# smolGura/fish-tts

Hardware: AMD Instinct MI355X
Metric: semantic tokens/sec (higher is better)
Workload: dtype bf16; 1 GPU; openaudio-s1-mini shapes (BASELINE configs[1]): batch=1 per GPU, 48-token prompt, 215 frames (10 s), top-p sampling, hipGraph-captured frame step, + DAC codec decode; prompt_len=48, parallelism=replica x1, frame_engine=3

## Files before the change

### fish-tts_amd/_lib.py

```python
from __future__ import annotations

import ctypes as C
import os
import subprocess

_HERE = os.path.dirname(os.path.abspath(__file__))
CSRC = os.path.join(_HERE, "csrc")
LIB_PATH = os.path.join(CSRC, "libfishtts_hip.so")

FT_OK = 0
FT_ERR_ARG, FT_ERR_HIP, FT_ERR_STATE, FT_ERR_UNSUPPORTED, FT_ERR_NOMEM, FT_ERR_TOO_LONG, FT_ERR_MISSING_WEIGHT = range(1, 8)
FT_F32, FT_BF16, FT_F16 = 0, 1, 2


class ft_ar_config(C.Structure):
    _fields_ = [(n, C.c_int32) for n in ("dtype", "vocab_size", "n_layer", "n_head", "dim", "intermediate_size",
                                         "n_local_heads", "head_dim")] + \
               [("rope_base", C.c_float), ("norm_eps", C.c_float)] + \
               [(n, C.c_int32) for n in ("max_seq_len", "tie_word_embeddings", "attention_qkv_bias", "attention_o_bias",
                                         "attention_qk_norm", "codebook_size", "num_codebooks",
                                         "scale_codebook_embeddings", "n_fast_layer", "fast_dim", "fast_n_head",
                                         "fast_n_local_heads", "fast_head_dim", "fast_intermediate_size",
                                         "fast_attention_qkv_bias", "fast_attention_qk_norm", "fast_attention_o_bias",
                                         "semantic_begin_id", "semantic_end_id", "im_end_id", "max_batch",
# ... 32 lines not shown
    "ft_ar_prefill_slow_many": (C.c_int32, [_P, C.c_int32, _P, _P, _P, _P]),
    "ft_ar_prefill_at": (C.c_int32, [_P, C.c_int32, _P, C.c_int32, C.c_int32, C.POINTER(ft_sampling), _P]),
    "ft_ar_kv_save": (C.c_int32, [_P, C.c_int32, C.c_int32, C.POINTER(_P)]),
    "ft_ar_kv_restore": (C.c_int32, [_P, _P, C.c_int32]),
    "ft_ar_kv_positions": (C.c_int32, [_P]),
    "ft_ar_kv_free": (None, [_P, _P]),
    "ft_ar_decode": (C.c_int32, [_P, C.c_int32, C.c_int32, C.POINTER(ft_sampling), C.c_int32, _P, _P]),
    "ft_ar_set_noise": (C.c_int32, [_P, _P, C.c_int64, C.c_int64]),
    "ft_ar_get_debug": (C.c_int32, [_P, C.c_int32, _P, _P]),
    "ft_codec_decode": (C.c_int32, [_P, _P, C.c_int32, C.c_int32, _P, _P]),
    "ft_codec_frame_len": (C.c_int32, [_P]),
    "ft_codec_stream_begin": (C.c_int32, [_P, C.POINTER(_P)]),
    "ft_codec_stream_decode": (C.c_int32, [_P, _P, _P, C.c_int32, _P]),
    "ft_codec_stream_end": (None, [_P, _P]),
    "ft_codec_stream_decode_many": (C.c_int32, [_P, C.c_int32, _P, _P, _P, _P]),
    "ft_resample_filter": (C.c_int32, [C.c_int32, _P, _P, _P, _P]),
    "ft_resampled_len": (C.c_int64, [C.c_int32, C.c_int64]),
    "ft_codec_decode_at": (C.c_int32, [_P, _P, C.c_int32, C.c_int32, _P, C.c_int32, _P, _P]),
    "ft_codec_stream_begin_at": (C.c_int32, [_P, C.c_int32, C.POINTER(_P)]),
    "ft_codec_stream_decode_many_at": (C.c_int32, [_P, C.c_int32, _P, _P, _P, _P, _P, _P]),
    "ft_test_resample": (C.c_int32, [_P, _P, C.c_int64, C.c_int32, _P, _P]),
    "ft_codec_encode": (C.c_int32, [_P, _P, C.c_int64, _P, _P]),
    "ft_codec_enc_frame_len": (C.c_int32, [_P]),
    "ft_codec_rvq_encode": (C.c_int32, [_P, _P, C.c_int32, _P]),
    "ft_ar_profile_gemv": (C.c_int32, [_P, C.c_int32, C.POINTER(ft_sampling), C.POINTER(C.c_double),
                                       C.POINTER(C.c_int64), C.POINTER(C.c_int64)]),
    "ft_ar_profile_frame": (C.c_int32, [_P, C.c_int32, C.POINTER(ft_sampling), C.POINTER(C.c_double), C.POINTER(C.c_double),
                                        C.POINTER(C.c_int32)]),
    "ft_sync": (C.c_int32, [_P]),
    "ft_ar_engine_state": (C.c_int32, [_P, _P, _P, _P]),
    "ft_ar_frame_path": (C.c_char_p, [_P]),
    "ft_test_engine_fault": (C.c_int32, [_P, C.c_int32, C.c_int32, C.c_int32]),
    "ft_test_sample": (C.c_int32, [_P, _P, C.c_int32, C.POINTER(ft_sampling), _P, _P, _P]),
    "ft_test_codec_trace_arm": (C.c_int32, [_P, C.c_int32, C.c_int32]),
    "ft_test_codec_trace_count": (C.c_int32, [_P]),
    "ft_test_codec_trace_variants": (C.c_int32, []),
    "ft_test_codec_trace_variant": (C.c_char_p, [C.c_int32, C.POINTER(C.c_int32), C.POINTER(C.c_int32)]),
    "ft_test_codec_trace_launch": (C.c_int32, [_P, C.c_int32, C.c_char_p, C.c_int32, C.POINTER(C.c_int32)]),
    "ft_test_codec_trace_buffer": (C.c_int32, [_P, C.c_int32, C.c_int32, C.POINTER(C.c_int32), C.POINTER(C.c_int32),
                                               C.POINTER(C.c_int64), _P]),
}

HIPCC_FLAGS = ["-O3", "--offload-arch=gfx950", "-ffp-contract=off", "-fPIC", "-shared", "-std=c++17",
               "-Wno-unused-value"]
SOURCES = ["engine.hip", "codec.hip"]


def _deps(path: str, seen=None) -> set:
    seen = set() if seen is None else seen
    path = os.path.normpath(path)
    if path in seen or not os.path.exists(path):
        return seen
    seen.add(path)
    with open(path) as f:
        for line in f:
            if line.startswith("#include \""):
                _deps(os.path.join(os.path.dirname(path), line.split('"')[1]), seen)
    return seen


def build(force: bool = False) -> str:
    hipcc = os.environ.get("HIPCC", "/opt/rocm/bin/hipcc")
    flags = [f for f in HIPCC_FLAGS if f != "-shared"]
    jobs, objs = [], []
    for s in SOURCES:
        src, obj = os.path.join(CSRC, s), os.path.join(CSRC, s.replace(".hip", ".o"))
# ... 35 lines not shown
```

### fish-tts_amd/ar_engine.py

```python
from __future__ import annotations

import ctypes as C
import logging
from typing import Dict, Iterator, List, Optional, Sequence

import numpy as np
import torch

from . import _lib as L
from .config import DualARModelArgs


class HipError(RuntimeError):
    pass


logger = logging.getLogger(__name__)


def _rope_table(n_pos: int, n_elem: int, base: float) -> torch.Tensor:
    expo = torch.arange(0, n_elem, 2)[: n_elem // 2].float() / n_elem
    inv_freq = 1.0 / (base ** expo)
    ang = torch.outer(torch.arange(n_pos), inv_freq)
    z = torch.polar(torch.ones_like(ang), ang)
# ... 201 lines not shown
        arr = (L.ft_sampling * ns)(*samplings)
        frames = np.zeros((ns, max(n_frames, 1), self.R), dtype=np.int32)
        n = np.zeros(ns, dtype=np.int32)
        self._check(self.lib.ft_ar_decode(self._h, ns, n_frames, arr, poll, frames.ctypes.data_as(C.c_void_p),
                                          n.ctypes.data_as(C.c_void_p)), "ft_ar_decode")
        return frames, n

    def set_noise(self, q: Optional[np.ndarray]):
        if q is None:
            self._check(self.lib.ft_ar_set_noise(self._h, None, 0, 0), "ft_ar_set_noise")
            return
        q = np.ascontiguousarray(q, dtype=np.float32)
        self._check(self.lib.ft_ar_set_noise(self._h, q.ctypes.data_as(C.c_void_p), q.shape[0], q.shape[1]),
                    "ft_ar_set_noise")

    def debug_state(self, slot: int = 0):
        logits = np.zeros(self.args.vocab_size, dtype=np.float32)
        hidden = np.zeros(self.args.fast_dim, dtype=np.float32)
        self._check(self.lib.ft_ar_get_debug(self._h, slot, logits.ctypes.data_as(C.c_void_p),
                                             hidden.ctypes.data_as(C.c_void_p)), "ft_ar_get_debug")
        return logits, hidden

    def test_sample(self, logits: np.ndarray, cb: int, sampling: L.ft_sampling, window=None, q=None) -> int:
        logits = np.ascontiguousarray(logits, dtype=np.float32)
        w = None if window is None else np.ascontiguousarray(window, dtype=np.int32)
        qq = None if q is None else np.ascontiguousarray(q, dtype=np.float32)
        out = np.zeros(1, dtype=np.int32)
        self._check(self.lib.ft_test_sample(
            self._h, logits.ctypes.data_as(C.c_void_p), cb, C.byref(sampling),
            None if w is None else w.ctypes.data_as(C.c_void_p),
            None if qq is None else qq.ctypes.data_as(C.c_void_p), out.ctypes.data_as(C.c_void_p)), "ft_test_sample")
        return int(out[0])

    def engine_state(self):
        f, a, w = C.c_int32(0), C.c_int32(0), C.c_int32(0)
        self._check(self.lib.ft_ar_engine_state(self._h, C.byref(f), C.byref(a), C.byref(w)), "ft_ar_engine_state")
        return f.value, a.value, w.value

    def sync(self):
        self._check(self.lib.ft_sync(self._h), "ft_sync")

    def profile_gemv(self, frames: int, sampling: L.ft_sampling):
        ms, n, b = C.c_double(), C.c_int64(), C.c_int64()
        self._check(self.lib.ft_ar_profile_gemv(self._h, frames, C.byref(sampling), C.byref(ms), C.byref(n),
                                                C.byref(b)), "ft_ar_profile_gemv")
        return ms.value, n.value, b.value

    def profile_frame(self, frames: int, sampling: L.ft_sampling):
        ms, n = C.c_double(0), C.c_int32(0)
        seg = (C.c_double * 3)()
        self._check(self.lib.ft_ar_profile_frame(self._h, frames, C.byref(sampling), C.byref(ms), seg, C.byref(n)),
                    "ft_ar_profile_frame")
        return ms.value, [seg[0], seg[1], seg[2]], n.value

    def _clamp_new(self, T: int, max_new_tokens: int) -> int:
        m = self.args.max_seq_len
        if T >= m:
            raise ValueError(f"Input sequence length {T} exceeds max_seq_len {m}")
        if max_new_tokens:
            if T + max_new_tokens > m:
                max_new_tokens = m - T
        else:
            max_new_tokens = m - T
        return min(max_new_tokens, self.max_new_tokens)

    def generate(self, prompt: np.ndarray, max_new_tokens: int, temperature: float = 0.7, top_p: float = 0.7,
# ... 45 lines not shown
```

### fish-tts_amd/csrc/ar_kernels.h

```cpp
#pragma once
#include "common.h"

namespace ft {

enum { PRO_NONE = 0, PRO_RMSNORM = 1 };
enum { EPI_STORE = 0, EPI_RESID = 1, EPI_SWIGLU = 2 };

__device__ __host__ __forceinline__ size_t xo_index(int m, int k, int ldm) { return ((size_t)(k >> 3) * ldm + m) * 8 + (k & 7); }

struct GemvP {
    const void* W;
    const void* bias;
    const float* x;
    int ldx;
    const void* gain;
    float eps;
    float* out;
    int ldo;
    const float* resid;
    int ldr;
    int N, K;
    int pro, epi;
    int nt;
};
// ... 1416 lines not shown
        const float* qrow = nullptr;
        if (p.noise && nfv < p.noise_rows) qrow = p.noise + (size_t)nfv * p.noise_row_len + p.noise_off;
        float q4[4];
        draw_noise4(p, ctl, qrow, i0, nfv, m, V, q4);
        ArgMax best{-1.f, 0x7fffffff};
#pragma unroll
        for (int e = 0; e < 4; ++e) {
            if (i0 + e < V) {
                const float prob = keep[e] ? rb<ROUND>(et[e] / Z2) : 0.f;
                best = better(best, ArgMax{rb<ROUND>(prob / rb<ROUND>(q4[e])), i0 + e});
            }
        }
        winner = block_best(best).i;
    }
    __syncthreads();
    finish_draw<WT>(p, m, winner, nfv);
}

struct SampCut {
    unsigned kstar;
    int nk;
    int all_kept;
    int argmax;
    float Lmax, Mt, Z2, Tc;
};

struct SampBigP {
    SampP s;
    SampCut* cut;
    int* chunk_cnt;
    float* part_score;
    int* part_idx;
    int nchunk;
};

__device__ __forceinline__ float key16_value(unsigned k16) {
    const uint32_t k = k16 << 16;
    const uint32_t u = (k & 0x80000000u) ? (k & 0x7fffffffu) : ~(k | 0xffffu);
    return __uint_as_float(u);
}

constexpr int SAMP_TH_THREADS = 1024;
constexpr int SAMP_TH_ROW = 33;
constexpr int SAMP_TH_OVF = 8;
constexpr size_t SAMP_TH_LDS = (size_t)SAMP_TH_THREADS * SAMP_TH_ROW * 4;

struct SampThShared {
    float red[16];
    int redi[16];
    float wsum[16];
    int wact[16];
    int AL[1024];
    unsigned ovf_key[SAMP_TH_OVF];
    unsigned ovf_cnt[SAMP_TH_OVF];
    int ovf_n;
    SampCut cut_s;
};

__device__ __forceinline__ void samp_cut_from_image(const SampBigP& b, const int m, const uint32_t* cimg, SampThShared& sh,
                                                    const bool has, const int kmax_t) {
    const SampP& p = b.s;
    const int tid = threadIdx.x, lane = tid & 63, wave = tid >> 6;
    const RowCtl ctl = p.ctl[m];
    float* red = sh.red;
    int* redi = sh.redi;
    float* wsum = sh.wsum;
    int* wact = sh.wact;
    int* AL = sh.AL;
    unsigned* ovf_key = sh.ovf_key;
    unsigned* ovf_cnt = sh.ovf_cnt;
    int& ovf_n = sh.ovf_n;
    SampCut& cut_s = sh.cut_s;
    const unsigned long long hb = __ballot(has);
    if (lane == 0) wact[wave] = __popcll(hb);
    __syncthreads();
    int abase = 0, n_active = 0;
    for (int w = 0; w < 16; ++w) { if (w < wave) abase += wact[w]; n_active += wact[w]; }
    if (has) AL[abase + __popcll(hb & ((1ull << lane) - 1ull))] = tid;
    ArgMax km = block_argmax(ArgMax{(float)kmax_t, tid}, red, redi);
    const unsigned kmax = (unsigned)(int)km.v;
    const float Lmax = key16_value(kmax);
    const int n_items = n_active * 64;
    const int ipt = (n_items + 1023) / 1024;
    const int i0 = tid * ipt, i1 = min(i0 + ipt, n_items);
    auto item_count = [&](int i, unsigned& k) -> float {
        const int g = AL[i >> 6], j = i & 63;
        k = 64u * g + j;
        const uint32_t w = cimg[g * SAMP_TH_ROW + (j >> 1)];
        unsigned c = (j & 1) ? (w >> 16) : (w & 0xffffu);
        if (c == 65535u)
            for (int q = 0; q < ovf_n && q < SAMP_TH_OVF; ++q) if (ovf_key[q] == k) c = ovf_cnt[q];
        return (float)c;
    };
    float z = 0.f;
    for (int i = i0; i < i1; ++i) {
        unsigned k;
        const float c = item_count(i, k);
        if (c > 0.f) z = fmaf(c, expf(key16_value(k) - Lmax), z);
    }
    const float Z = block_sum(z, red);
    const float tp = round_bf16(ctl.top_p);
    auto removed = [&](float cum) { return round_bf16(cum) > tp; };
    auto prob = [&](unsigned k16) { return round_bf16(expf(key16_value(k16) - Lmax) / Z); };
    float mt = 0.f;
    for (int i = i0; i < i1; ++i) {
        unsigned k;
        const float c = item_count(i, k);
        if (c > 0.f) mt = fmaf(c, prob(k), mt);
    }
    float suf = mt;
#pragma unroll
    for (int o = 1; o < 64; o <<= 1) {
        const float t = __shfl_down(suf, o, 64);
        if (lane + o < 64) suf += t;
    }
    __syncthreads();
    if (lane == 0) wsum[wave] = suf;
    __syncthreads();
    float above = suf - mt;
    for (int w = wave + 1; w < 16; ++w) above += wsum[w];
    int found = -1;
    unsigned f_key = 0;
    float f_above = 0.f, f_cnt = 0.f;
    float run = above;
    for (int i = i1 - 1; i >= i0; --i) {
        unsigned k;
        const float c = item_count(i, k);
        if (c > 0.f) {
            const float nxt = fmaf(c, prob(k), run);
            if (found < 0 && removed(nxt)) { found = i; f_key = k; f_above = run; f_cnt = c; }
            run = nxt;
        }
    }
    ArgMax who = block_argmax(ArgMax{found >= 0 ? (float)tid : -1.f, tid}, red, redi);
    if (tid == 0) { cut_s.all_kept = who.v < 0.f ? 1 : 0; cut_s.kstar = 0; cut_s.nk = 0; }
    __syncthreads();
    if (who.v >= 0.f && tid == (int)who.v) {
        const float pk = prob(f_key);
        int lo_n = 0, hi_n = (int)f_cnt;
        while (lo_n < hi_n) {
            const int mid = (lo_n + hi_n + 1) >> 1;
            if (removed(fmaf((float)mid, pk, f_above))) hi_n = mid - 1; else lo_n = mid;
        }
        if (f_key == kmax && lo_n < 1) lo_n = 1;
        cut_s.kstar = f_key;
        cut_s.nk = lo_n;
    }
    __syncthreads();
    const unsigned kstar = cut_s.kstar;
    const int nk = cut_s.nk, all_kept = cut_s.all_kept;
    const float Tc = fmaxf(ctl.temperature, 1e-5f);
    const float Mt = round_bf16(Lmax / Tc);
    float z2 = 0.f;
    for (int i = i0; i < i1; ++i) {
        unsigned k;
        const float c = item_count(i, k);
        if (c > 0.f) {
            float n = 0.f;
            if (all_kept || k > kstar) n = c;
            else if (k == kstar) n = (float)nk;
            if (n > 0.f) z2 = fmaf(n, expf(round_bf16(key16_value(k) / Tc) - Mt), z2);
        }
    }
    const float Z2 = block_sum(z2, red);
    if (tid == 0) {
        SampCut o;
        o.kstar = kstar; o.nk = nk; o.all_kept = all_kept; o.argmax = 0;
        o.Lmax = Lmax; o.Mt = Mt; o.Z2 = Z2; o.Tc = Tc;
        b.cut[m] = o;
    }
}

static __global__ __launch_bounds__(1024) void samp_cut_kernel(SampBigP b) {
    extern __shared__ __attribute__((aligned(16))) uint32_t cimg[];
    __shared__ SampThShared sh;
    __shared__ int pen_id[32];
    __shared__ float pen_val[32];
    const SampP& p = b.s;
    const int m = blockIdx.x, tid = threadIdx.x;
    float* L = p.logits + (size_t)m * p.ldl;
    const int V = p.V;
    const RowCtl ctl = p.ctl[m];
    const int nfv = p.nf[m];
    const int R = p.ncb + 1;
    const int* seq = p.seq + (size_t)m * R * p.cap;
    for (int i = tid; i < SAMP_TH_THREADS * SAMP_TH_ROW; i += 1024) cimg[i] = 0u;
    if (tid == 0) sh.ovf_n = 0;
    const int npen = nfv > 0 ? (p.cb == 0 ? R : 16) : 0;
    auto count1 = [&](float v) {
        const unsigned k = order_key(v) >> 16;
        atomicAdd(&cimg[(k >> 6) * SAMP_TH_ROW + ((k & 63u) >> 1)], (k & 1u) ? 0x10000u : 1u);
    };
    {
        if (nfv > 0) {
            const int it = nfv - 1;
            const int ws = it < 16 ? 0 : it - 16;
            if (tid < npen) {
                const int id = p.cb == 0 ? seq[(size_t)tid * p.cap + ws + 1] : seq[(size_t)(p.cb + 1) * p.cap + ws + 1 + tid];
                pen_id[tid] = -1;
                if (id >= 0 && id < V) {
                    const float sv = L[id];
                    pen_id[tid] = id;
                    pen_val[tid] = sv < 0.f ? round_bf16(sv * ctl.rep) : round_bf16(sv / ctl.rep);
                }
            }
            __syncthreads();
            if (tid < npen && pen_id[tid] >= 0) L[pen_id[tid]] = pen_val[tid];
        }
        if (p.cb == 0 && ctl.ban_eos && tid == 0 && p.im_end < V) L[p.im_end] = -INFINITY;
        __syncthreads();
        const int V16 = ((reinterpret_cast<uintptr_t>(L) & 15) == 0) ? (V / 16384) * 16384 : 0;
        float4 fa[4], fb[4];
        auto ld16 = [&](float4 (&f)[4], int base) {
#pragma unroll
            for (int u = 0; u < 4; ++u) f[u] = *reinterpret_cast<const float4*>(L + base + u * 4096 + tid * 4);
        };
        auto cnt16 = [&](const float4 (&f)[4]) {
#pragma unroll
            for (int u = 0; u < 4; ++u) { count1(f[u].x); count1(f[u].y); count1(f[u].z); count1(f[u].w); }
        };
        if (V16 > 0) ld16(fa, 0);
        for (int base = 0; base < V16; base += 32768) {
            if (base + 16384 < V16) ld16(fb, base + 16384);
            cnt16(fa);
            if (base + 32768 < V16) ld16(fa, base + 32768);
            if (base + 16384 < V16) cnt16(fb);
        }
        for (int base = V16; base < V; base += 4096) {
            float f[4];
#pragma unroll
            for (int u = 0; u < 4; ++u) { const int i = base + u * 1024 + tid; f[u] = i < V ? L[i] : 0.f; }
#pragma unroll
            for (int u = 0; u < 4; ++u) if (base + u * 1024 + tid < V) count1(f[u]);
        }
    }
    __syncthreads();
    const uint32_t* row = cimg + tid * SAMP_TH_ROW;
    int kmax_t = -1;
    unsigned tot = 0;
#pragma unroll 8
    for (int j = 0; j < 32; ++j) {
        const uint32_t w = row[j];
        const unsigned c0 = w & 0xffffu, c1 = w >> 16;
        if (c0) kmax_t = 64 * tid + 2 * j;
        if (c1) kmax_t = 64 * tid + 2 * j + 1;
        tot += c0 + c1;
    }
    const int total = (int)block_sum((float)tot, sh.red);
    if (total != V) {
        __shared__ unsigned exc_key[SAMP_TH_OVF];
        __shared__ unsigned exc_cnt[SAMP_TH_OVF];
        for (int i = tid; i < SAMP_TH_THREADS * SAMP_TH_ROW; i += 1024) cimg[i] = 0u;
        if (tid < SAMP_TH_OVF) { exc_key[tid] = 0xffffffffu; exc_cnt[tid] = 0u; }
        __syncthreads();
        for (int i = tid; i < V; i += 1024) {
            const unsigned k = order_key(L[i]) >> 16;
            uint32_t* d = &cimg[(k >> 6) * SAMP_TH_ROW + ((k & 63u) >> 1)];
            const unsigned shft = (k & 1u) * 16u;
            for (;;) {
                const uint32_t old = *reinterpret_cast<volatile uint32_t*>(d);
                if (((old >> shft) & 0xffffu) == 65535u) {
                    for (int q = 0; q < SAMP_TH_OVF; ++q) {
                        const unsigned prev = atomicCAS(&exc_key[q], 0xffffffffu, k);
                        if (prev == 0xffffffffu || prev == k) { atomicAdd(&exc_cnt[q], 1u); break; }
                    }
                    break;
                }
                if (atomicCAS(d, old, old + (1u << shft)) == old) break;
            }
        }
        __syncthreads();
        if (tid == 0) {
            int n = 0;
            for (int q = 0; q < SAMP_TH_OVF; ++q)
                if (exc_key[q] != 0xffffffffu) { sh.ovf_key[n] = exc_key[q]; sh.ovf_cnt[n] = 65535u + exc_cnt[q]; ++n; }
            sh.ovf_n = n;
        }
        kmax_t = -1;
        tot = 0;
        for (int j = 0; j < 32; ++j) {
            const uint32_t w = row[j];
            if (w & 0xffffu) kmax_t = 64 * tid + 2 * j;
            if (w >> 16) kmax_t = 64 * tid + 2 * j + 1;
            tot += (w & 0xffffu) + (w >> 16);
        }
        __syncthreads();
    }
    samp_cut_from_image(b, m, cimg, sh, tot != 0u, kmax_t);
}

static __global__ __launch_bounds__(256) void samp_count_kernel(SampBigP b) {
    __shared__ float red[4];
    const SampP& p = b.s;
    const int m = blockIdx.y, tid = threadIdx.x;
    const int c0 = blockIdx.x * 1024;
    const float* L = p.logits + (size_t)m * p.ldl;
    const SampCut cut = b.cut[m];
    float c = 0.f;
#pragma unroll
    for (int e = 0; e < 4; ++e) {
        const int i = c0 + 4 * tid + e;
        if (i < p.V && (order_key(L[i]) >> 16) == cut.kstar) c += 1.f;
    }
    c = wave_sum(c);
    if ((tid & 63) == 0) red[tid >> 6] = c;
    __syncthreads();
    if (tid == 0) b.chunk_cnt[(size_t)m * b.nchunk + blockIdx.x] = (int)(red[0] + red[1] + red[2] + red[3]);
}

static __global__ __launch_bounds__(256) void samp_race_kernel(SampBigP b) {
    __shared__ float red[4];
    __shared__ int redi[4];
    __shared__ int wcnt[4];
    const SampP& p = b.s;
    const int m = blockIdx.y, tid = threadIdx.x, lane = tid & 63, wave = tid >> 6;
    const int c0 = blockIdx.x * 1024;
    const float* L = p.logits + (size_t)m * p.ldl;
    const int V = p.V;
    const RowCtl ctl = p.ctl[m];
    const int nfv = p.nf[m];
// ... 74 lines not shown
```

### fish-tts_amd/csrc/engine.h

```cpp
#pragma once
#include <hip/hip_runtime.h>

#include <map>
#include <string>
#include <vector>

#include "../../include/fishtts_hip.h"
#include "../../include/fishtts_hip_test.h"
#include "common.h"

namespace ft {
struct RowCtl;
struct SampCut;
struct EngLayer;
}

struct FtTensor {
    void* p = nullptr;
    std::vector<int64_t> shape;
    int dtype = FT_BF16;
    int64_t numel() const {
        int64_t n = 1;
        for (auto s : shape) n *= s;
        return n;
// ... 28 lines not shown
    std::vector<FtLayer> layers, flayers;

    float *x = nullptr, *qkv = nullptr, *y = nullptr, *g = nullptr, *logits = nullptr, *hid = nullptr,
          *femb = nullptr, *xf = nullptr, *qkvf = nullptr, *gf = nullptr, *flog = nullptr, *part_o = nullptr,
          *part_ml = nullptr;
    int n_slots = 0, nsplit = 1, cap = 0, fastV = 0, y_ld = 0;
    int nsplit_max = 1;
    bool nsplit_fixed = false;
    float *pf_x = nullptr, *pf_qkv = nullptr, *pf_y = nullptr;
    ft::bf16_t *pf_xn = nullptr, *pf_ybf = nullptr, *pf_g = nullptr, *pf_qbf = nullptr;
    int4* pf_seqs = nullptr;
    int2* pf_rows = nullptr;
    ft::bf16_t *xo_x = nullptr, *xo_xf = nullptr, *xo_femb = nullptr, *xo_y = nullptr, *xo_g = nullptr;
    ft::bf16_t* wide_qkv0_tab = nullptr;
    int xo_ldm = 0;
    int xo_pair = 0;
    bool no_attn_wide = false;
    bool no_head_stream = false;
    bool no_pair = false;
    int wide_min = 5;
    bool wide_ok = false;
    bool prefill_v0 = false;
    int prefill_gemm_mode = 2;
    size_t cache_m_stride = 0, fcache_m_stride = 0;

    int *d_pos = nullptr, *d_tok = nullptr, *d_tokn = nullptr, *d_seq = nullptr, *d_nf = nullptr,
        *d_done = nullptr, *d_prompt = nullptr;
    ft::RowCtl* d_ctl = nullptr;
    int *h_pin = nullptr;
    float* noise = nullptr;
    long noise_rows = 0, noise_row_len = 0;

    ft::SampCut* samp_cut = nullptr;
    int* samp_chunk_cnt = nullptr;
    float* samp_part_score = nullptr;
    int* samp_part_idx = nullptr;

    bool eng_on = false;
    bool eng_fast_on = false;
    int eng_nb = 0;
    ft::EngLayer *eng_layers = nullptr, *eng_flayers = nullptr;
    unsigned *eng_gx = nullptr, *eng_gqkv = nullptr, *eng_gy = nullptr, *eng_gxb = nullptr, *eng_gg = nullptr;
    unsigned long long* eng_gpart = nullptr;
    unsigned* eng_fast_g = nullptr;
    unsigned* eng_ctl = nullptr;
    size_t eng_lds_slow = 0, eng_lds_fast = 0, eng_fast_words = 0, eng_pool_words = 0;
    bool eng_relay = true;
    void* eng_qkv0_tab = nullptr;
    bool eng_pair = false;
    bool xl_shape = false;
    bool eng_xl = false;
    std::string path_str;
    const void* eng_slow_fn = nullptr;
    const void* eng_fast_fn = nullptr;
    size_t eng_pool_bytes = 0, eng_gpart_bytes = 0, eng_fast_bytes = 0;
    bool eng_suspended = false;
    int eng_strikes = 0, eng_last_where = 0;
    bool eng_owner = false;
    std::string eng_why;

    std::map<int, hipGraphExec_t> graphs;
    std::map<int, int> graph_nodes;

    bool prof = false, prof_count_only = false;
    std::vector<hipEvent_t> prof_ev;
    int64_t prof_bytes = 0, prof_launches = 0;
// ... 18 lines not shown
```

### fish-tts_amd/csrc/engine.hip

```cpp
#include "engine.h"
#include "ar_kernels.h"
#include "frame_engine.h"
#include "wide_kernels.h"
#include "codec_kernels.h"

#include <math.h>

#include <algorithm>
#include <mutex>
#include <stdio.h>
#include <stdlib.h>
#include <string.h>

using namespace ft;

static std::string g_create_err;
static void eng_release(ft_ctx* ctx);

ft_status ft_fail(ft_ctx* ctx, ft_status code, const std::string& msg) {
    if (ctx) ctx->err = msg; else g_create_err = msg;
    return code;
}

template <typename S, typename D>
// ... 156 lines not shown
    if (!ctx->prefill_v0) {
        const size_t S = c.max_seq_len;
        FT_TRY(dmalloc(ctx, &ctx->pf_x, S * c.dim));
        FT_TRY(dmalloc(ctx, &ctx->pf_qkv, S * qkvN));
        FT_TRY(dmalloc(ctx, &ctx->pf_y, S * c.n_head * c.head_dim));
        FT_TRY(dmalloc(ctx, &ctx->pf_xn, S * c.dim));
        FT_TRY(dmalloc(ctx, &ctx->pf_ybf, S * c.n_head * c.head_dim));
        FT_TRY(dmalloc(ctx, &ctx->pf_g, S * c.intermediate_size));
        FT_TRY(dmalloc(ctx, &ctx->pf_qbf, S * c.n_head * c.head_dim));
        FT_TRY(dmalloc(ctx, &ctx->pf_seqs, M));
        FT_TRY(dmalloc(ctx, &ctx->pf_rows, S));
    }
    if (c.dtype == FT_F16 || !ctx->prefill_v0) {
        const int HD = c.n_head * c.head_dim, HDf = c.fast_n_head * c.fast_head_dim;
        ctx->wide_ok = !getenv("FT_NO_WIDE") && !c.fast_attention_qkv_bias && !c.fast_attention_o_bias && c.fast_dim == c.dim &&
                       wide_k_ok(c.dim) && wide_k_ok(HD) && wide_k_ok(c.intermediate_size) && wide_k_ok(HDf) && wide_k_ok(c.fast_intermediate_size) &&
                       qkvN % 32 == 0 && fqkvN % 32 == 0 && c.intermediate_size % 16 == 0 && c.fast_intermediate_size % 16 == 0 &&
                       c.dim % 16 == 0 && c.vocab_size % 32 == 0 && ctx->fastV % 16 == 0;
        if (ctx->wide_ok) {
            ctx->xo_pair = (int)((M + 15) / 16 * 16);
            ctx->no_pair = getenv("FT_NO_PAIR") != nullptr;
            ctx->no_attn_wide = getenv("FT_NO_ATTN_WIDE") != nullptr;
            ctx->no_head_stream = getenv("FT_NO_HEAD_STREAM") != nullptr;
            ctx->xo_ldm = 2 * ctx->xo_pair;
            const size_t P = ctx->xo_ldm;
            FT_TRY(dmalloc(ctx, &ctx->xo_x, P * c.dim));
            FT_TRY(dmalloc(ctx, &ctx->xo_xf, P * c.fast_dim));
            FT_TRY(dmalloc(ctx, &ctx->xo_femb, P * c.fast_dim));
            FT_TRY(dmalloc(ctx, &ctx->xo_y, P * (size_t)std::max(HD, HDf)));
            FT_TRY(dmalloc(ctx, &ctx->xo_g, P * (size_t)std::max(c.intermediate_size, c.fast_intermediate_size)));
        }
    }
    const size_t nchunk = ((size_t)c.vocab_size + 1023) / 1024;
    FT_TRY(dmalloc(ctx, &ctx->samp_cut, M));
    FT_TRY(dmalloc(ctx, &ctx->samp_chunk_cnt, M * nchunk));
    FT_TRY(dmalloc(ctx, &ctx->samp_part_score, M * nchunk));
    FT_TRY(dmalloc(ctx, &ctx->samp_part_idx, M * nchunk));
    FT_HIP(ctx, hipHostMalloc((void**)&ctx->h_pin, (3 * M + 8) * sizeof(int), hipHostMallocDefault));
    return FT_OK;
}

extern "C" ft_status ft_create(const ft_ar_config* ar, const ft_codec_config* codec, int32_t device, ft_ctx** out) {
    if (!out || (!ar && !codec)) return ft_fail(nullptr, FT_ERR_ARG, "ft_create: need a config and an out pointer");
    int ndev = 0;
    if (hipGetDeviceCount(&ndev) != hipSuccess || ndev == 0)
        return ft_fail(nullptr, FT_ERR_HIP, "ft_create: no HIP device visible (the MI355X path has no CPU fallback)");
    if (device < 0 || device >= ndev) return ft_fail(nullptr, FT_ERR_ARG, "ft_create: bad device index");
    ft_ctx* ctx = new ft_ctx();
    ctx->device = device;
    ft_status st = FT_OK;
    do {
        if (hipSetDevice(device) != hipSuccess) { st = ft_fail(ctx, FT_ERR_HIP, "hipSetDevice failed"); break; }
        if (hipStreamCreateWithFlags(&ctx->stream, hipStreamNonBlocking) != hipSuccess) {
            st = ft_fail(ctx, FT_ERR_HIP, "hipStreamCreate failed"); break;
        }
        if (ar) {
            ctx->c = *ar;
            ctx->has_ar = true;
            if ((st = ar_validate(ctx)) != FT_OK) break;
            if ((st = ar_alloc(ctx)) != FT_OK) break;
            ar_expected(ctx);
        }
        if (codec) {
            ctx->cc = *codec;
            ctx->has_codec = true;
            if ((st = codec_create(ctx)) != FT_OK) break;
// ... 842 lines not shown
template <typename WT, int ROUND>
static void enqueue_sample(Launch& L, int cb, bool last) {
    if (L.gemv_only) return;
    ft_ctx* ctx = L.ctx;
    const ft_ar_config& c = ctx->c;
    const int m0 = L.m0, R = c.num_codebooks + 1;
    SampP s{};
    if (cb == 0) { s.logits = ctx->logits + (size_t)m0 * c.vocab_size; s.ldl = c.vocab_size; s.V = c.vocab_size; }
    else { s.logits = ctx->flog + (size_t)m0 * ctx->fastV; s.ldl = ctx->fastV; s.V = ctx->fastV; }
    s.ctl = ctx->d_ctl + m0; s.tokn = ctx->d_tokn + (size_t)m0 * R; s.seq = ctx->d_seq + (size_t)m0 * R * ctx->cap;
    s.cap = ctx->cap; s.nf = ctx->d_nf + m0; s.cb = cb; s.ncb = c.num_codebooks; s.sem_begin = c.semantic_begin_id;
    s.im_end = c.im_end_id; s.cbsize = c.codebook_size; s.fast_emb = ctx->fast_emb;
    s.femb = ctx->femb + (size_t)m0 * c.fast_dim; s.Df = c.fast_dim; s.noise = ctx->noise;
    s.noise_row_len = ctx->noise_row_len; s.noise_rows = ctx->noise_rows;
    s.noise_off = cb == 0 ? 0 : (long)c.vocab_size + (long)(cb - 1) * ctx->fastV;
    s.last = last ? 1 : 0; s.tok = ctx->d_tok + (size_t)m0 * R; s.pos = ctx->d_pos + m0; s.done = ctx->d_done + m0;
    if (wide_batch(L)) {
        s.femb_xo = (cb == 0 && wide_pair(L) ? ctx->xo_x + (size_t)ctx->xo_pair * 8 : ctx->xo_femb) + (size_t)m0 * 8;
        s.femb_ldm = ctx->xo_ldm;
        if (cb >= 1 && cb + 1 < c.num_codebooks && ctx->wide_qkv0_tab) {
            s.qkv0_tab = ctx->wide_qkv0_tab; s.qkv0_n = (c.fast_n_head + 2 * c.fast_n_local_heads) * c.fast_head_dim;
            s.qkv0_out = ctx->qkvf + (size_t)m0 * s.qkv0_n;
        }
    }
    if (s.V <= 1024) {
        sample_small_kernel<WT, ROUND><<<L.M, 256, 0, L.s>>>(s);
    } else if (ROUND == RND_BF16) {
        SampBigP b{};
        b.s = s; b.nchunk = (s.V + 1023) / 1024;
        b.cut = ctx->samp_cut + m0;
        b.chunk_cnt = ctx->samp_chunk_cnt + (size_t)m0 * b.nchunk;
        b.part_score = ctx->samp_part_score + (size_t)m0 * b.nchunk;
        b.part_idx = ctx->samp_part_idx + (size_t)m0 * b.nchunk;
        const dim3 gridc(b.nchunk, L.M);
        {
            static DevOnce once;
            once.run([] {
                hipFuncSetAttribute((const void*)samp_cut_kernel, hipFuncAttributeMaxDynamicSharedMemorySize, (int)SAMP_TH_LDS);
            });
        }
        samp_cut_kernel<<<L.M, SAMP_TH_THREADS, SAMP_TH_LDS, L.s>>>(b);
        samp_count_kernel<<<gridc, 256, 0, L.s>>>(b);
        samp_race_kernel<<<gridc, 256, 0, L.s>>>(b);
        samp_finish_kernel<WT><<<L.M, 256, 0, L.s>>>(b);
    } else {
        sample_block_kernel<WT, ROUND><<<L.M, 1024, 0, L.s>>>(s);
    }
    L.chk();
}

template <typename WT, int ROUND>
static void enqueue_fast_step(Launch& L, const int cb, const bool pair = false) {
    ft_ctx* ctx = L.ctx;
    const ft_ar_config& c = ctx->c;
    const int m0 = L.m0;
    const int Df = c.fast_dim, Hf = c.fast_n_head, Hkvf = c.fast_n_local_heads, hdf = c.fast_head_dim;
    const size_t qkvN = (size_t)(Hf + 2 * Hkvf) * hdf;
    float* xf = ctx->xf + (size_t)m0 * Df;
    float* qkvf = ctx->qkvf + (size_t)m0 * qkvN;
    float* gf = ctx->gf + (size_t)m0 * c.fast_intermediate_size;
    {
        const float* xin = cb == 0 ? ctx->hid + (size_t)m0 * Df : ctx->femb + (size_t)m0 * Df;
        const bool wide = wide_batch(L);
        for (int li = 0; li < c.n_fast_layer; ++li) {
            const FtLayer& l = ctx->flayers[li];
            const float* xl = li == 0 ? xin : xf;
// ... 992 lines not shown
    FT_HIP(ctx, hipMemcpy(cb == 0 ? ctx->logits : ctx->flog, logits, (size_t)V * sizeof(float), hipMemcpyHostToDevice));
    int nfv = 0;
    if (window) {
        nfv = 1;
        for (int r = 0; r < R; ++r)
            FT_HIP(ctx, hipMemcpy(ctx->d_seq + (size_t)r * ctx->cap + 1, window + (size_t)r * 16, 16 * sizeof(int), hipMemcpyHostToDevice));
        FT_HIP(ctx, hipMemcpy(ctx->d_nf, &nfv, sizeof(int), hipMemcpyHostToDevice));
    }
    float* saved = ctx->noise;
    const long srows = ctx->noise_rows, slen = ctx->noise_row_len;
    float* tmp = nullptr;
    if (q) {
        const long need = (long)c.vocab_size + (long)(c.num_codebooks - 1) * ctx->fastV;
        FT_HIP(ctx, hipMalloc((void**)&tmp, (size_t)(nfv + 1) * need * sizeof(float)));
        const long off = cb == 0 ? 0 : (long)c.vocab_size + (long)(cb - 1) * ctx->fastV;
        FT_HIP(ctx, hipMemcpy(tmp + (size_t)nfv * need + off, q, (size_t)V * sizeof(float), hipMemcpyHostToDevice));
        ctx->noise = tmp; ctx->noise_rows = nfv + 1; ctx->noise_row_len = need;
    } else {
        ctx->noise = nullptr; ctx->noise_rows = 0;
    }
    Launch L{ctx, ctx->stream, 0, 1, 0};
    if (c.dtype == FT_BF16) enqueue_sample<bf16_t, RND_BF16>(L, cb, false);
    else if (c.dtype == FT_F16) enqueue_sample<f16_t, RND_F16>(L, cb, false);
    else enqueue_sample<float, RND_NONE>(L, cb, false);
    hipError_t e = hipStreamSynchronize(ctx->stream);
    ctx->noise = saved; ctx->noise_rows = srows; ctx->noise_row_len = slen;
    if (tmp) hipFree(tmp);
    if (L.err != hipSuccess || e != hipSuccess) return ft_fail(ctx, FT_ERR_HIP, "ft_test_sample launch failed");
    int tokn[2] = {0, 0};
    FT_HIP(ctx, hipMemcpy(tokn, ctx->d_tokn + (cb == 0 ? 0 : cb + 1), sizeof(int), hipMemcpyDeviceToHost));
    *out_index = tokn[0];
    return ft_ar_reset(ctx, 0);
}
```

Before: 775.2 tokens/s.

## Keep top-p cut histogram items in registers and apply repetition penalty late

The top-p cut kernel now caches each thread's histogram counts, keys and probabilities in registers, so later passes do not recompute them from shared memory and recompute expf. The full vocabulary is loaded with vector loads even when its length is not a multiple of 16384. The repetition penalty and EOS ban are applied after the histogram is built, by moving individual counts, which lets the first logit load overlap the penalty-id fetch. The change adds register pressure and a recount fallback when a count underflows or overflows, plus optional timestamp hooks and a test entry point. An environment variable turns the new paths off.

```diff
diff --git a/fish-tts_amd/_lib.py b/fish-tts_amd/_lib.py
--- a/fish-tts_amd/_lib.py
+++ b/fish-tts_amd/_lib.py
@@ -88,6 +88,7 @@
     "ft_ar_frame_path": (C.c_char_p, [_P]),
     "ft_test_engine_fault": (C.c_int32, [_P, C.c_int32, C.c_int32, C.c_int32]),
     "ft_test_sample": (C.c_int32, [_P, _P, C.c_int32, C.POINTER(ft_sampling), _P, _P, _P]),
+    "ft_test_sample_cut": (C.c_int32, [_P, _P, C.POINTER(ft_sampling), _P, C.c_int32, _P, _P, _P]),
     "ft_test_codec_trace_arm": (C.c_int32, [_P, C.c_int32, C.c_int32]),
     "ft_test_codec_trace_count": (C.c_int32, [_P]),
     "ft_test_codec_trace_variants": (C.c_int32, []),
diff --git a/fish-tts_amd/ar_engine.py b/fish-tts_amd/ar_engine.py
--- a/fish-tts_amd/ar_engine.py
+++ b/fish-tts_amd/ar_engine.py
@@ -257,6 +257,20 @@
             None if qq is None else qq.ctypes.data_as(C.c_void_p), out.ctypes.data_as(C.c_void_p)), "ft_test_sample")
         return int(out[0])
 
+    def test_sample_cut(self, logits: np.ndarray, sampling: L.ft_sampling, hist=None, q=None):
+        logits = np.ascontiguousarray(logits, dtype=np.float32)
+        h = None if hist is None else np.ascontiguousarray(hist, dtype=np.int32)
+        nf = 0 if h is None else int(h.shape[1])
+        qq = None if q is None else np.ascontiguousarray(q, dtype=np.float32)
+        out = np.zeros(1, dtype=np.int32)
+        cut = np.zeros(8, dtype=np.int32)
+        self._check(self.lib.ft_test_sample_cut(
+            self._h, logits.ctypes.data_as(C.c_void_p), C.byref(sampling),
+            None if h is None or nf == 0 else h.ctypes.data_as(C.c_void_p), nf,
+            None if qq is None else qq.ctypes.data_as(C.c_void_p), out.ctypes.data_as(C.c_void_p),
+            cut.ctypes.data_as(C.c_void_p)), "ft_test_sample_cut")
+        return int(out[0]), cut
+
     def engine_state(self):
         f, a, w = C.c_int32(0), C.c_int32(0), C.c_int32(0)
         self._check(self.lib.ft_ar_engine_state(self._h, C.byref(f), C.byref(a), C.byref(w)), "ft_ar_engine_state")
diff --git a/fish-tts_amd/csrc/ar_kernels.h b/fish-tts_amd/csrc/ar_kernels.h
--- a/fish-tts_amd/csrc/ar_kernels.h
+++ b/fish-tts_amd/csrc/ar_kernels.h
@@ -1472,7 +1472,16 @@
     float* part_score;
     int* part_idx;
     int nchunk;
+    int cut_flags;
+    unsigned long long* stamps;
 };
+constexpr int SAMP_CUT_REUSE = 1;
+constexpr int SAMP_CUT_VTAIL = 2;
+constexpr int SAMP_CUT_LATEPEN = 4;
+constexpr int SAMP_CUT_ALL = SAMP_CUT_REUSE | SAMP_CUT_VTAIL | SAMP_CUT_LATEPEN;
+constexpr int SAMP_CUT_IPT = 16;
+constexpr int SAMP_STAMPS = 16;
+#define SAMP_STAMP(k) do { if (b.stamps && threadIdx.x == 0) b.stamps[(size_t)blockIdx.x * SAMP_STAMPS + (k)] = __builtin_amdgcn_s_memrealtime(); } while (0)
 
 __device__ __forceinline__ float key16_value(unsigned k16) {
     const uint32_t k = k16 << 16;
@@ -1532,22 +1541,52 @@
             for (int q = 0; q < ovf_n && q < SAMP_TH_OVF; ++q) if (ovf_key[q] == k) c = ovf_cnt[q];
         return (float)c;
     };
+    const bool reg = (b.cut_flags & SAMP_CUT_REUSE) && ipt <= SAMP_CUT_IPT;
+    float cv[SAMP_CUT_IPT], pv[SAMP_CUT_IPT];
+    unsigned kv[SAMP_CUT_IPT];
+    SAMP_STAMP(6);
     float z = 0.f;
-    for (int i = i0; i < i1; ++i) {
-        unsigned k;
-        const float c = item_count(i, k);
-        if (c > 0.f) z = fmaf(c, expf(key16_value(k) - Lmax), z);
-    }
+    if (reg) {
+#pragma unroll
+        for (int j = 0; j < SAMP_CUT_IPT; ++j) {
+            cv[j] = 0.f; pv[j] = 0.f; kv[j] = 0u;
+            if (j < ipt && i0 + j < i1) {
+                cv[j] = item_count(i0 + j, kv[j]);
+                if (cv[j] > 0.f) { pv[j] = expf(key16_value(kv[j]) - Lmax); z = fmaf(cv[j], pv[j], z); }
+            }
+        }
+    } else {
+        for (int i = i0; i < i1; ++i) {
+            unsigned k;
+            const float c = item_count(i, k);
+            if (c > 0.f) z = fmaf(c, expf(key16_value(k) - Lmax), z);
+        }
+    }
+    auto hold = [&]() {
+        if (reg) {
+#pragma unroll
+            for (int j = 0; j < SAMP_CUT_IPT; ++j) asm volatile("" : "+v"(cv[j]), "+v"(pv[j]), "+v"(kv[j]));
+        }
+    };
+    hold();
     const float Z = block_sum(z, red);
+    SAMP_STAMP(7);
     const float tp = round_bf16(ctl.top_p);
     auto removed = [&](float cum) { return round_bf16(cum) > tp; };
     auto prob = [&](unsigned k16) { return round_bf16(expf(key16_value(k16) - Lmax) / Z); };
     float mt = 0.f;
-    for (int i = i0; i < i1; ++i) {
-        unsigned k;
-        const float c = item_count(i, k);
-        if (c > 0.f) mt = fmaf(c, prob(k), mt);
-    }
+    if (reg) {
+#pragma unroll
+        for (int j = 0; j < SAMP_CUT_IPT; ++j)
+            if (cv[j] > 0.f) { pv[j] = round_bf16(pv[j] / Z); mt = fmaf(cv[j], pv[j], mt); }
+    } else {
+        for (int i = i0; i < i1; ++i) {
+            unsigned k;
+            const float c = item_count(i, k);
+            if (c > 0.f) mt = fmaf(c, prob(k), mt);
+        }
+    }
+    hold();
     float suf = mt;
 #pragma unroll
     for (int o = 1; o < 64; o <<= 1) {
@@ -1559,24 +1598,37 @@
     __syncthreads();
     float above = suf - mt;
     for (int w = wave + 1; w < 16; ++w) above += wsum[w];
+    SAMP_STAMP(8);
     int found = -1;
     unsigned f_key = 0;
-    float f_above = 0.f, f_cnt = 0.f;
+    float f_above = 0.f, f_cnt = 0.f, f_p = 0.f;
     float run = above;
-    for (int i = i1 - 1; i >= i0; --i) {
-        unsigned k;
-        const float c = item_count(i, k);
-        if (c > 0.f) {
-            const float nxt = fmaf(c, prob(k), run);
-            if (found < 0 && removed(nxt)) { found = i; f_key = k; f_above = run; f_cnt = c; }
-            run = nxt;
-        }
-    }
+    if (reg) {
+#pragma unroll
+        for (int j = SAMP_CUT_IPT - 1; j >= 0; --j) {
+            if (cv[j] > 0.f) {
+                const float nxt = fmaf(cv[j], pv[j], run);
+                if (found < 0 && removed(nxt)) { found = i0 + j; f_key = kv[j]; f_above = run; f_cnt = cv[j]; f_p = pv[j]; }
+                run = nxt;
+            }
+        }
+    } else {
+        for (int i = i1 - 1; i >= i0; --i) {
+            unsigned k;
+            const float c = item_count(i, k);
+            if (c > 0.f) {
+                const float nxt = fmaf(c, prob(k), run);
+                if (found < 0 && removed(nxt)) { found = i; f_key = k; f_above = run; f_cnt = c; }
+                run = nxt;
+            }
+        }
+    }
+    hold();
     ArgMax who = block_argmax(ArgMax{found >= 0 ? (float)tid : -1.f, tid}, red, redi);
     if (tid == 0) { cut_s.all_kept = who.v < 0.f ? 1 : 0; cut_s.kstar = 0; cut_s.nk = 0; }
     __syncthreads();
     if (who.v >= 0.f && tid == (int)who.v) {
-        const float pk = prob(f_key);
+        const float pk = reg ? f_p : prob(f_key);
         int lo_n = 0, hi_n = (int)f_cnt;
         while (lo_n < hi_n) {
             const int mid = (lo_n + hi_n + 1) >> 1;
@@ -1587,28 +1639,38 @@
         cut_s.nk = lo_n;
     }
     __syncthreads();
+    SAMP_STAMP(9);
     const unsigned kstar = cut_s.kstar;
     const int nk = cut_s.nk, all_kept = cut_s.all_kept;
     const float Tc = fmaxf(ctl.temperature, 1e-5f);
     const float Mt = round_bf16(Lmax / Tc);
     float z2 = 0.f;
-    for (int i = i0; i < i1; ++i) {
-        unsigned k;
-        const float c = item_count(i, k);
-        if (c > 0.f) {
-            float n = 0.f;
-            if (all_kept || k > kstar) n = c;
-            else if (k == kstar) n = (float)nk;
-            if (n > 0.f) z2 = fmaf(n, expf(round_bf16(key16_value(k) / Tc) - Mt), z2);
+    auto kept_term = [&](float c, unsigned k) {
+        float n = 0.f;
+        if (all_kept || k > kstar) n = c;
+        else if (k == kstar) n = (float)nk;
+        if (n > 0.f) z2 = fmaf(n, expf(round_bf16(key16_value(k) / Tc) - Mt), z2);
+    };
+    if (reg) {
+#pragma unroll
+        for (int j = 0; j < SAMP_CUT_IPT; ++j)
+            if (cv[j] > 0.f) kept_term(cv[j], kv[j]);
+    } else {
+        for (int i = i0; i < i1; ++i) {
+            unsigned k;
+            const float c = item_count(i, k);
+            if (c > 0.f) kept_term(c, k);
         }
     }
     const float Z2 = block_sum(z2, red);
+    SAMP_STAMP(10);
     if (tid == 0) {
         SampCut o;
         o.kstar = kstar; o.nk = nk; o.all_kept = all_kept; o.argmax = 0;
         o.Lmax = Lmax; o.Mt = Mt; o.Z2 = Z2; o.Tc = Tc;
         b.cut[m] = o;
     }
+    if (b.stamps && tid == 0) { asm volatile("s_waitcnt vmcnt(0)" ::: "memory"); SAMP_STAMP(11); }
 }
 
 static __global__ __launch_bounds__(1024) void samp_cut_kernel(SampBigP b) {
@@ -1616,6 +1678,7 @@
     __shared__ SampThShared sh;
     __shared__ int pen_id[32];
     __shared__ float pen_val[32];
+    __shared__ int pen_recount;
     const SampP& p = b.s;
     const int m = blockIdx.x, tid = threadIdx.x;
     float* L = p.logits + (size_t)m * p.ldl;
@@ -1624,57 +1687,102 @@
     const int nfv = p.nf[m];
     const int R = p.ncb + 1;
     const int* seq = p.seq + (size_t)m * R * p.cap;
-    for (int i = tid; i < SAMP_TH_THREADS * SAMP_TH_ROW; i += 1024) cimg[i] = 0u;
-    if (tid == 0) sh.ovf_n = 0;
+    SAMP_STAMP(0);
     const int npen = nfv > 0 ? (p.cb == 0 ? R : 16) : 0;
+    const bool ban = p.cb == 0 && ctl.ban_eos && p.im_end < V;
     auto count1 = [&](float v) {
         const unsigned k = order_key(v) >> 16;
         atomicAdd(&cimg[(k >> 6) * SAMP_TH_ROW + ((k & 63u) >> 1)], (k & 1u) ? 0x10000u : 1u);
     };
-    {
+    auto pen_seq_id = [&]() {
+        const int ws = nfv - 1 < 16 ? 0 : nfv - 1 - 16;
+        const int id = p.cb == 0 ? seq[(size_t)tid * p.cap + ws + 1] : seq[(size_t)(p.cb + 1) * p.cap + ws + 1 + tid];
+        return id >= 0 && id < V ? id : -1;
+    };
+    auto penalised = [&](float sv) { return sv < 0.f ? round_bf16(sv * ctl.rep) : round_bf16(sv / ctl.rep); };
+    const bool al16 = (reinterpret_cast<uintptr_t>(L) & 15) == 0;
+    const int V16 = al16 ? (V / 16384) * 16384 : 0;
+    const int VW = ((b.cut_flags & SAMP_CUT_VTAIL) && al16 && (V & 3) == 0) ? V : V16;
+    float4 fa[4], fb[4];
+    auto ld16 = [&](float4 (&f)[4], int base) {
+#pragma unroll
+        for (int u = 0; u < 4; ++u) {
+            const int i = base + u * 4096 + tid * 4;
+            f[u] = i < VW ? *reinterpret_cast<const float4*>(L + i) : float4{0.f, 0.f, 0.f, 0.f};
+        }
+    };
+    auto cnt16 = [&](const float4 (&f)[4], int base) {
+#pragma unroll
+        for (int u = 0; u < 4; ++u)
+            if (base + u * 4096 + tid * 4 < VW) { count1(f[u].x); count1(f[u].y); count1(f[u].z); count1(f[u].w); }
+    };
+    const bool late = (b.cut_flags & SAMP_CUT_LATEPEN) != 0;
+    int my_id = -1;
+    float my_old = 0.f, eos_old = 0.f;
+    if (late) {
+        if (tid < npen) my_id = pen_seq_id();
+        if (VW > 0) ld16(fa, 0);
+    }
+    for (int i = tid; i < SAMP_TH_THREADS * SAMP_TH_ROW; i += 1024) cimg[i] = 0u;
+    if (tid == 0) { sh.ovf_n = 0; pen_recount = 0; }
+    SAMP_STAMP(1);
+    if (late) {
+        if (tid < npen) pen_id[tid] = my_id;
+        __syncthreads();
+        if (my_id >= 0) my_old = L[my_id];
+        if (ban && tid == 0) eos_old = L[p.im_end];
+    } else {
         if (nfv > 0) {
-            const int it = nfv - 1;
-            const int ws = it < 16 ? 0 : it - 16;
             if (tid < npen) {
-                const int id = p.cb == 0 ? seq[(size_t)tid * p.cap + ws + 1] : seq[(size_t)(p.cb + 1) * p.cap + ws + 1 + tid];
-                pen_id[tid] = -1;
-                if (id >= 0 && id < V) {
-                    const float sv = L[id];
-                    pen_id[tid] = id;
-                    pen_val[tid] = sv < 0.f ? round_bf16(sv * ctl.rep) : round_bf16(sv / ctl.rep);
-                }
+                const int id = pen_seq_id();
+                pen_id[tid] = id;
+                if (id >= 0) pen_val[tid] = penalised(L[id]);
             }
             __syncthreads();
             if (tid < npen && pen_id[tid] >= 0) L[pen_id[tid]] = pen_val[tid];
         }
-        if (p.cb == 0 && ctl.ban_eos && tid == 0 && p.im_end < V) L[p.im_end] = -INFINITY;
+        if (ban && tid == 0) L[p.im_end] = -INFINITY;
         __syncthreads();
-        const int V16 = ((reinterpret_cast<uintptr_t>(L) & 15) == 0) ? (V / 16384) * 16384 : 0;
-        float4 fa[4], fb[4];
-        auto ld16 = [&](float4 (&f)[4], int base) {
-#pragma unroll
-            for (int u = 0; u < 4; ++u) f[u] = *reinterpret_cast<const float4*>(L + base + u * 4096 + tid * 4);
+        if (VW > 0) ld16(fa, 0);
+    }
+    SAMP_STAMP(2);
+    for (int base = 0; base < VW; base += 32768) {
+        if (base + 16384 < VW) ld16(fb, base + 16384);
+        cnt16(fa, base);
+        if (base + 32768 < VW) ld16(fa, base + 32768);
+        if (base + 16384 < VW) cnt16(fb, base + 16384);
+    }
+    SAMP_STAMP(3);
+    for (int base = VW; base < V; base += 4096) {
+        float f[4];
+#pragma unroll
+        for (int u = 0; u < 4; ++u) { const int i = base + u * 1024 + tid; f[u] = i < V ? L[i] : 0.f; }
+#pragma unroll
+        for (int u = 0; u < 4; ++u) if (base + u * 1024 + tid < V) count1(f[u]);
+    }
+    __syncthreads();
+    SAMP_STAMP(4);
+    if (late) {
+        auto move1 = [&](float from, float to) {
+            const unsigned kf = order_key(from) >> 16, kt = order_key(to) >> 16;
+            const uint32_t of = atomicSub(&cimg[(kf >> 6) * SAMP_TH_ROW + ((kf & 63u) >> 1)], (kf & 1u) ? 0x10000u : 1u);
+            if (((kf & 1u) ? (of >> 16) : (of & 0xffffu)) == 0u) pen_recount = 1;
+            const uint32_t ot = atomicAdd(&cimg[(kt >> 6) * SAMP_TH_ROW + ((kt & 63u) >> 1)], (kt & 1u) ? 0x10000u : 1u);
+            if (((kt & 1u) ? (ot >> 16) : (ot & 0xffffu)) == 65535u) pen_recount = 1;
         };
-        auto cnt16 = [&](const float4 (&f)[4]) {
-#pragma unroll
-            for (int u = 0; u < 4; ++u) { count1(f[u].x); count1(f[u].y); count1(f[u].z); count1(f[u].w); }
-        };
-        if (V16 > 0) ld16(fa, 0);
-        for (int base = 0; base < V16; base += 32768) {
-            if (base + 16384 < V16) ld16(fb, base + 16384);
-            cnt16(fa);
-            if (base + 32768 < V16) ld16(fa, base + 32768);
-            if (base + 16384 < V16) cnt16(fb);
-        }
-        for (int base = V16; base < V; base += 4096) {
-            float f[4];
-#pragma unroll
-            for (int u = 0; u < 4; ++u) { const int i = base + u * 1024 + tid; f[u] = i < V ? L[i] : 0.f; }
-#pragma unroll
-            for (int u = 0; u < 4; ++u) if (base + u * 1024 + tid < V) count1(f[u]);
-        }
-    }
-    __syncthreads();
+        if (my_id >= 0 && !(ban && my_id == p.im_end)) {
+            bool first = true;
+            for (int t = 0; t < tid; ++t) first = first && pen_id[t] != my_id;
+            if (first) {
+                const float nv = penalised(my_old);
+                move1(my_old, nv);
+                L[my_id] = nv;
+            }
+        }
+        if (ban && tid == 0) { move1(eos_old, -INFINITY); L[p.im_end] = -INFINITY; }
+        __syncthreads();
+        SAMP_STAMP(12);
+    }
     const uint32_t* row = cimg + tid * SAMP_TH_ROW;
     int kmax_t = -1;
     unsigned tot = 0;
@@ -1687,7 +1795,7 @@
         tot += c0 + c1;
     }
     const int total = (int)block_sum((float)tot, sh.red);
-    if (total != V) {
+    if (total != V || pen_recount) {
         __shared__ unsigned exc_key[SAMP_TH_OVF];
         __shared__ unsigned exc_cnt[SAMP_TH_OVF];
         for (int i = tid; i < SAMP_TH_THREADS * SAMP_TH_ROW; i += 1024) cimg[i] = 0u;
@@ -1726,6 +1834,7 @@
         }
         __syncthreads();
     }
+    SAMP_STAMP(5);
     samp_cut_from_image(b, m, cimg, sh, tot != 0u, kmax_t);
 }
 
diff --git a/fish-tts_amd/csrc/engine.h b/fish-tts_amd/csrc/engine.h
--- a/fish-tts_amd/csrc/engine.h
+++ b/fish-tts_amd/csrc/engine.h
@@ -84,6 +84,7 @@
     long noise_rows = 0, noise_row_len = 0;
 
     ft::SampCut* samp_cut = nullptr;
+    int samp_cut_flags = 0;
     int* samp_chunk_cnt = nullptr;
     float* samp_part_score = nullptr;
     int* samp_part_idx = nullptr;
diff --git a/fish-tts_amd/csrc/engine.hip b/fish-tts_amd/csrc/engine.hip
--- a/fish-tts_amd/csrc/engine.hip
+++ b/fish-tts_amd/csrc/engine.hip
@@ -212,6 +212,7 @@
         }
     }
     const size_t nchunk = ((size_t)c.vocab_size + 1023) / 1024;
+    ctx->samp_cut_flags = getenv("FT_NO_CUT_REUSE") ? 0 : SAMP_CUT_ALL;
     FT_TRY(dmalloc(ctx, &ctx->samp_cut, M));
     FT_TRY(dmalloc(ctx, &ctx->samp_chunk_cnt, M * nchunk));
     FT_TRY(dmalloc(ctx, &ctx->samp_part_score, M * nchunk));
@@ -1120,6 +1121,7 @@
         b.chunk_cnt = ctx->samp_chunk_cnt + (size_t)m0 * b.nchunk;
         b.part_score = ctx->samp_part_score + (size_t)m0 * b.nchunk;
         b.part_idx = ctx->samp_part_idx + (size_t)m0 * b.nchunk;
+        b.cut_flags = ctx->samp_cut_flags;
         const dim3 gridc(b.nchunk, L.M);
         {
             static DevOnce once;
@@ -2178,3 +2180,43 @@
     *out_index = tokn[0];
     return ft_ar_reset(ctx, 0);
 }
+
+extern "C" ft_status ft_test_sample_cut(ft_ctx* ctx, const float* logits, const ft_sampling* sp, const int32_t* hist, int32_t nf,
+                                        const float* q, int32_t* out_index, int32_t* cut) {
+    FT_TRY(ar_ready(ctx));
+    const ft_ar_config& c = ctx->c;
+    if (!logits || !sp || !out_index || !cut || nf < 0 || nf + 1 >= ctx->cap || (nf > 0 && !hist))
+        return ft_fail(ctx, FT_ERR_ARG, "ft_test_sample_cut: bad argument");
+    if (c.dtype != FT_BF16 || c.vocab_size <= 1024) return ft_fail(ctx, FT_ERR_UNSUPPORTED, "ft_test_sample_cut: not the large-vocabulary bf16 draw");
+    const int R = c.num_codebooks + 1;
+    const int V = c.vocab_size;
+    FT_TRY(ft_ar_reset(ctx, 0));
+    FT_TRY(upload_ctl(ctx, 0, 1, sp));
+    FT_HIP(ctx, hipMemcpy(ctx->logits, logits, (size_t)V * sizeof(float), hipMemcpyHostToDevice));
+    if (nf > 0) {
+        for (int r = 0; r < R; ++r)
+            FT_HIP(ctx, hipMemcpy(ctx->d_seq + (size_t)r * ctx->cap + 1, hist + (size_t)r * nf, (size_t)nf * sizeof(int), hipMemcpyHostToDevice));
+        FT_HIP(ctx, hipMemcpy(ctx->d_nf, &nf, sizeof(int), hipMemcpyHostToDevice));
+    }
+    float* saved = ctx->noise;
+    const long srows = ctx->noise_rows, slen = ctx->noise_row_len;
+    float* tmp = nullptr;
+    if (q) {
+        const long need = (long)c.vocab_size + (long)(c.num_codebooks - 1) * ctx->fastV;
+        FT_HIP(ctx, hipMalloc((void**)&tmp, (size_t)(nf + 1) * need * sizeof(float)));
+        FT_HIP(ctx, hipMemcpy(tmp + (size_t)nf * need, q, (size_t)V * sizeof(float), hipMemcpyHostToDevice));
+        ctx->noise = tmp; ctx->noise_rows = nf + 1; ctx->noise_row_len = need;
+    } else {
+        ctx->noise = nullptr; ctx->noise_rows = 0;
+    }
+    Launch L{ctx, ctx->stream, 0, 1, 0};
+    enqueue_sample<bf16_t, RND_BF16>(L, 0, false);
+    hipError_t e = hipStreamSynchronize(ctx->stream);
+    ctx->noise = saved; ctx->noise_rows = srows; ctx->noise_row_len = slen;
+    if (tmp) hipFree(tmp);
+    if (L.err != hipSuccess || e != hipSuccess) return ft_fail(ctx, FT_ERR_HIP, "ft_test_sample_cut launch failed");
+    static_assert(sizeof(SampCut) == 8 * sizeof(int32_t), "SampCut is read back as 8 words");
+    FT_HIP(ctx, hipMemcpy(cut, ctx->samp_cut, sizeof(SampCut), hipMemcpyDeviceToHost));
+    FT_HIP(ctx, hipMemcpy(out_index, ctx->d_tokn, sizeof(int), hipMemcpyDeviceToHost));
+    return ft_ar_reset(ctx, 0);
+}
```

Result: no change. 775.1 tokens/s (median of 2 runs) (-0.0%).
